# carkod/binquant

Hardware: AMD Instinct MI355X
Metric: symbol-candles/s for full indicator set (14 fp64 columns) (higher is better)
Workload: dtype f64; 1 GPU; configs[3]: 100000 symbols x 10000 candles, symbol-sharded over 1 GPU(s) (100000 symbols x 10000 candles on rank 0); symbols=100000, symbols_per_gpu=100000, candles=10000, parallelism=symbol-sharded x1, no data-path collective

## Files before the change

### binquant_amd/csrc/bq_device.h

```cpp
#pragma once
#include <hip/hip_runtime.h>
#include <math.h>
#include <stdint.h>

namespace bq {

constexpr int WAVE = 64;

__device__ __forceinline__ double qnan() { return __builtin_nan(""); }

__device__ __forceinline__ double win_val(double x) { return x - x == 0.0 ? x : qnan(); }
__device__ __forceinline__ bool win_ok(double x) { return x - x == 0.0; }

__device__ __forceinline__ uint64_t order_key(double v) {
  const uint64_t u = (uint64_t)__double_as_longlong(v);
  return (u >> 63) ? ~u : (u | 0x8000000000000000ull);
}

__device__ __forceinline__ double key_value(uint64_t k) {
  const uint64_t u = (k >> 63) ? (k & 0x7fffffffffffffffull) : ~k;
  return __longlong_as_double((long long)u);
}

struct dd {
// ... 115 lines not shown
__device__ __forceinline__ int wave_scan_max_dpp(int x, int lane) {
  x = max(x, dpp_i32<DPP_ROW_SHR1>(x));
  x = max(x, dpp_i32<DPP_ROW_SHR2>(x));
  x = max(x, dpp_i32<DPP_ROW_SHR4>(x));
  x = max(x, dpp_i32<DPP_ROW_SHR8>(x));
  const int r0 = __builtin_amdgcn_readlane(x, 15);
  const int r1 = max(r0, __builtin_amdgcn_readlane(x, 31));
  const int r2 = max(r1, __builtin_amdgcn_readlane(x, 47));
  const int row = lane >> 4;
  const int c = row == 0 ? 0 : (row == 1 ? r0 : (row == 2 ? r1 : r2));
  return max(x, c);
}

template <int NB>
__device__ __forceinline__ double pow_bits(const double* apow, int n) {
  double r = 1.0;
#pragma unroll
  for (int j = 0; j < NB; ++j)
    if (n & (1 << j)) r *= apow[j];
  return r;
}

__device__ __forceinline__ double wave_scan_affine_dpp(double b, const double* apow, int lane) {
  b = fma(apow[0], dpp_f64<DPP_ROW_SHR1>(b), b);
  b = fma(apow[1], dpp_f64<DPP_ROW_SHR2>(b), b);
  b = fma(apow[2], dpp_f64<DPP_ROW_SHR4>(b), b);
  b = fma(apow[3], dpp_f64<DPP_ROW_SHR8>(b), b);
  const double c1 = readlane_f64(b, 15);
  const double c2 = fma(apow[4], c1, readlane_f64(b, 31));
  const double c3 = fma(apow[4], c2, readlane_f64(b, 47));
  const int row = lane >> 4;
  if (row > 0) {
    const double c = row == 1 ? c1 : (row == 2 ? c2 : c3);
    b = fma(pow_bits<5>(apow, (lane & 15) + 1), c, b);
  }
  return b;
}

__device__ __forceinline__ double wave_scan_affine_dpp_rp(double b, const double* apow, double rp, int lane) {
  b = fma(apow[0], dpp_f64<DPP_ROW_SHR1>(b), b);
  b = fma(apow[1], dpp_f64<DPP_ROW_SHR2>(b), b);
  b = fma(apow[2], dpp_f64<DPP_ROW_SHR4>(b), b);
  b = fma(apow[3], dpp_f64<DPP_ROW_SHR8>(b), b);
  const double c1 = readlane_f64(b, 15);
  const double c2 = fma(apow[4], c1, readlane_f64(b, 31));
  const double c3 = fma(apow[4], c2, readlane_f64(b, 47));
  const int row = lane >> 4;
  if (row > 0) {
    const double c = row == 1 ? c1 : (row == 2 ? c2 : c3);
    b = fma(rp, c, b);
  }
  return b;
}

__device__ __forceinline__ double gain_of(double d) { return d > 0.0 ? d : 0.0; }
__device__ __forceinline__ double loss_of(double d) { return d < 0.0 ? -d : 0.0; }

__device__ __forceinline__ double true_range(double h, double l, double pc) {
  double a = h - l;
  double b = fabs(h - pc);
  double c = fabs(l - pc);
  return fmax(a, fmax(b, c));
}

__device__ __forceinline__ double ohlc4(double o, double h, double l, double c) {
  return (((o + h) + l) + c) / 4.0;
}

__device__ __forceinline__ double typical_price(double h, double l, double c) {
  return ((h + l) + c) / 3.0;
}

__device__ __forceinline__ double oscillator(double a, double b) {
  return (100.0 * a) / (a + b);
}

__device__ __forceinline__ double div_exact(double x, double n, double r) {
  double q = x * r;
  const double e = fma(-q, n, x);
  return fma(e, r, q);
}

__device__ __forceinline__ double div_count(double x, double n, double r) {
  if (__builtin_expect(fabs(x) < 0x1p-960 && x != 0.0, 0)) return x / n;
  const double q = x * r;
  const double c = fma(fma(-q, n, x), r, q);
  return ((x == 0.0) | !(fabs(q) <= __DBL_MAX__)) ? q : c;
}

__device__ __forceinline__ double rcp_nr(double v) {
  double r = __builtin_amdgcn_rcp(v);
  r = fma(r, fma(-v, r, 1.0), r);
  return fma(r, fma(-v, r, 1.0), r);
}

__device__ __forceinline__ double log_return(double c, double p) {
  const double m = c / p;
  const double d = m - 1.0;
  if (__builtin_expect(!(fabs(d) <= 0.125), 0)) return log(m);
  const double s = d * rcp_nr(2.0 + d), z = s * s;
  double r = 1.0 / 15.0;
  r = fma(r, z, 1.0 / 13.0);
  r = fma(r, z, 1.0 / 11.0);
  r = fma(r, z, 1.0 / 9.0);
  r = fma(r, z, 1.0 / 7.0);
  r = fma(r, z, 1.0 / 5.0);
  r = fma(r, z, 1.0 / 3.0);
  return (2.0 * s) * fma(r, z, 1.0);
}

__device__ __forceinline__ double sqrt_nr(double v) {
  const double r = __builtin_amdgcn_rsq(v);
  const double s = v * r;
  const double h = 0.5 * r;
  const double e = fma(-s, s, v);
  const double q = fma(h, e, s);
  return v > 0.0 ? q : 0.0;
}

constexpr int STG_PITCH = WAVE + 2;

typedef unsigned int bq_u32x2 __attribute__((__vector_size__(8)));

template <int CT>
__device__ __forceinline__ void stage_load(const double* __restrict__ base, int64_t ld, int64_t sym0, int64_t S,
                                           int t0, int T, int lane, double (&r)[CT]) {
#pragma unroll
  for (int k = 0; k < CT; ++k) {
    const int e = lane + WAVE * k;
    const int64_t s = sym0 + e / CT;
    const int t = t0 + e % CT;
    const int64_t sc = s < S ? s : S - 1;
    const int tc = t < 0 ? 0 : t < T ? t : T - 1;
    const double v = base[sc * ld + tc];
    r[k] = (s < S && t >= 0 && t < T) ? v : qnan();
  }
}

template <int CT>
__device__ __forceinline__ void stage_put(double* lds, int lane, const double (&r)[CT]) {
#pragma unroll
  for (int k = 0; k < CT; ++k) {
    const int e = lane + WAVE * k;
    lds[(e % CT) * STG_PITCH + e / CT] = r[k];
  }
}

template <int CT, typename OutT>
__device__ __forceinline__ void stage_store(const double* lds, OutT* __restrict__ base, int64_t ld, int64_t sym0,
                                            int64_t S, int t0, int T, int lane) {
  const int64_t rows = S - sym0 < WAVE ? S - sym0 : WAVE;
  const int nbytes = base ? (int)(rows * ld * (int64_t)sizeof(OutT)) : 0;
  const __amdgpu_buffer_rsrc_t rs =
      __builtin_amdgcn_make_buffer_rsrc(base ? base + sym0 * ld : nullptr, 0, nbytes, 0x00020000);
#pragma unroll
  for (int k = 0; k < CT; ++k) {
    const int e = lane + WAVE * k;
    const int r = e / CT;
    const int t = t0 + e % CT;
    const bool ok = r < rows && t < T;
    const unsigned off = ok ? (unsigned)(((int64_t)r * ld + t) * (int64_t)sizeof(OutT)) : (unsigned)nbytes;
    const double v = lds[(e % CT) * STG_PITCH + r];
    if constexpr (sizeof(OutT) == 1)
      __builtin_amdgcn_raw_buffer_store_b8((unsigned char)(OutT)v, rs, off, 0, 0);
    else
      __builtin_amdgcn_raw_buffer_store_b64(__builtin_bit_cast(bq_u32x2, (double)(OutT)v), rs, off, 0, 0);
  }
}

__device__ __forceinline__ int lower_bound_i64(const int64_t* __restrict__ ts, int n, int64_t key) {
  int lo = 0, hi = n;
  while (lo < hi) {
    const int mid = (lo + hi) >> 1;
    if (ts[mid] < key) lo = mid + 1;
    else hi = mid;
  }
  return lo;
}

__device__ __forceinline__ int lower_bound_guess(const int64_t* __restrict__ ts, int n, int64_t key, int64_t t0v,
                                                 int64_t step) {
  if (step > 0) {
    int64_t g = key <= t0v ? 0 : (key - t0v + step - 1) / step;
    g = g > n ? n : g;
    const bool ok = (g == 0 || ts[g - 1] < key) && (g == n || ts[g] >= key);
    if (ok) return (int)g;
  }
  return lower_bound_i64(ts, n, key);
}

__device__ __forceinline__ double safe_pct(double cur, double prev) {
  if (prev == 0.0) return 0.0;
  return (cur - prev) / fabs(prev);
}


typedef double dbl2 __attribute__((ext_vector_type(2)));

union DwordsOf2 {
  dbl2 d;
  unsigned u[4];
};

__device__ __forceinline__ void swap_halves(dbl2& a, dbl2& b) {
  DwordsOf2 x, y;
  x.d = a;
  y.d = b;
#pragma unroll
  for (int i = 0; i < 4; ++i) {
    const auto r = __builtin_amdgcn_permlane32_swap(x.u[i], y.u[i], false, false);
    x.u[i] = r[0];
    y.u[i] = r[1];
  }
  a = x.d;
  b = y.d;
}

__device__ __forceinline__ void swap_rows(dbl2& a, dbl2& b) {
  DwordsOf2 x, y;
  x.d = a;
  y.d = b;
#pragma unroll
  for (int i = 0; i < 4; ++i) {
    const auto r = __builtin_amdgcn_permlane16_swap(x.u[i], y.u[i], false, false);
    x.u[i] = r[0];
    y.u[i] = r[1];
  }
  a = x.d;
  b = y.d;
}

template <int K>
__device__ __forceinline__ void line_exchange(dbl2 (&p)[K / 2]) {
  static_assert(K == 4 || K == 8, "line_exchange: 4 or 8 candles per lane");
  if constexpr (K == 4) {
    swap_halves(p[0], p[1]);
  } else {
    swap_halves(p[0], p[2]);
    swap_halves(p[1], p[3]);
    swap_rows(p[0], p[1]);
    swap_rows(p[2], p[3]);
  }
}

template <int K>
__device__ __forceinline__ int line_offset(int lane) {
  if constexpr (K == 4) return lane < 32 ? 4 * lane : 4 * (lane - 32) + 2;
  else return 8 * (lane & 15) + 2 * (lane >> 4);
}


template <int K>
__device__ __forceinline__ void store_lines(double* __restrict__ row_, int tb, int T, bool vec, const double (&x)[K],
                                            bool full = false) {
  typedef __attribute__((address_space(1))) double gd;
  typedef __attribute__((address_space(1))) dbl2 gd2;
  gd* row = (gd*)row_;
  if (vec) {
    dbl2 p[K / 2];
#pragma unroll
    for (int j = 0; j < K / 2; ++j) p[j] = dbl2{x[2 * j], x[2 * j + 1]};
    line_exchange<K>(p);
    const int lane = __lane_id();
    const int t = tb - K * lane + line_offset<K>(lane);
#pragma unroll
    for (int m = 0; m < K / 2; ++m) {
      const int u = t + 128 * m;
      if (full || u + 2 <= T) __builtin_nontemporal_store(p[m], reinterpret_cast<gd2*>(row + u));
      else if (u < T) row[u] = p[m].x;
    }
  } else {
#pragma unroll
    for (int k = 0; k < K; ++k)
      if (tb + k < T) row[tb + k] = x[k];
  }
}


template <bool UNROLL, typename F>
__device__ __forceinline__ void walk_window(int lo, F&& f) {
  if constexpr (UNROLL) {
#pragma unroll
    for (int x = lo; x <= 0; ++x) f(x);
  } else {
    for (int x = lo; x <= 0; ++x) f(x);
  }
}


template <int K>
__device__ __forceinline__ void line_unexchange(dbl2 (&p)[K / 2]) {
  static_assert(K == 4 || K == 8, "line_unexchange: 4 or 8 candles per lane");
  if constexpr (K == 4) {
    swap_halves(p[0], p[1]);
  } else {
    swap_rows(p[0], p[1]);
    swap_rows(p[2], p[3]);
    swap_halves(p[0], p[2]);
    swap_halves(p[1], p[3]);
  }
}

template <int K>
__device__ __forceinline__ void load_pieces(const double* __restrict__ row, int tb, int T, double (&x)[K],
                                            double fill) {
  const int lane = __lane_id();
  const int t = tb - K * lane + line_offset<K>(lane);
#pragma unroll
  for (int m = 0; m < K / 2; ++m) {
    const int u = t + 128 * m;
    if (u + 2 <= T) {
      const dbl2 v = *reinterpret_cast<const dbl2*>(row + u);
      x[2 * m] = v.x;
      x[2 * m + 1] = v.y;
    } else {
      x[2 * m] = u < T ? row[u] : fill;
      x[2 * m + 1] = fill;
    }
  }
}

template <int K>
__device__ __forceinline__ void line_unexchange_x(double (&x)[K]) {
  dbl2 p[K / 2];
#pragma unroll
  for (int m = 0; m < K / 2; ++m) p[m] = dbl2{x[2 * m], x[2 * m + 1]};
  line_unexchange<K>(p);
#pragma unroll
  for (int m = 0; m < K / 2; ++m) {
    x[2 * m] = p[m].x;
    x[2 * m + 1] = p[m].y;
  }
}

}
```

### binquant_amd/csrc/bq_enrich.hip

```cpp
#include "bq_rowtile.h"
#include "binquant_amd.h"

#include <stddef.h>
#include <string.h>

#include <type_traits>

namespace bq {

#ifndef BQ_EN_NT
#define BQ_EN_NT 256
#endif
#ifndef BQ_EN_K
#define BQ_EN_K 4
#endif
#ifndef BQ_EN_NTSTORE
#define BQ_EN_NTSTORE 1
#endif
#ifndef BQ_EN_SWIZZLE
#define BQ_EN_SWIZZLE 0
#endif
#ifndef BQ_EN_WPS
#define BQ_EN_WPS 3
#endif
constexpr int EN_NT = BQ_EN_NT;
constexpr int EN_NW = EN_NT / WAVE;
constexpr int EN_K = BQ_EN_K;
constexpr int EN_TT = EN_NT * EN_K;
constexpr int EN_LK = EN_K == 2 ? 1 : EN_K == 4 ? 2 : 3;
constexpr int EN_H = 128;
constexpr int EN_R = EN_H + EN_TT;
static_assert(EN_K % 2 == 0 && EN_TT >= EN_H && EN_K * WAVE > BQ_MAX_WINDOW, "tile shape");

#ifndef BQ_EN_LDSPERM
#define BQ_EN_LDSPERM 1
#endif
#if BQ_EN_LDSPERM
#define LX(i) ((((i) & (EN_K - 1)) * (EN_R / EN_K)) + ((i) >> EN_LK))
#define RS(x) (lb + LX(x))
#define RS1(x) (pb / EN_K + LX(x))
#else
#define LX(i) (i)
#define RS(x) (pb + (x))
#define RS1(x) (pb + (x))
#endif
static_assert(!BQ_EN_LDSPERM || ((1 << EN_LK) == EN_K && EN_R % EN_K == 0), "LX: power-of-two candles per lane");

enum { E_FAST = 0, E_SLOW, E_SIG, E_0, E_1, NE };

struct Pow {
  double a0, a1, p, q, a2, a3, a4;
};

__host__ __device__ __forceinline__ Pow pow_mul(const Pow& T, const Pow& U) {
  Pow r;
  r.a0 = T.a0 * U.a0;
  r.a1 = T.a1 * U.a1;
  r.p = fma(T.p, U.a0, T.a2 * U.p);
  r.q = fma(T.q, U.a1, T.a2 * U.q);
  r.a2 = T.a2 * U.a2;
  r.a3 = T.a3 * U.a3;
  r.a4 = T.a4 * U.a4;
  return r;
}

struct EmaHost {
  double al[NE], om[NE], den[NE], la[NE], lb[NE];
  Pow step;
  Pow wstep[6];
  Pow wave[EN_NW + 1];
};

struct EnrichArgs {
  EmaHost ema;
  const double* in[BQ_NUM_INPUTS];
  double* out[BQ_NUM_ENRICH_COLS];
  int64_t ld_in, ld_out;
  int64_t S, swz;
  int T;
  int ma[3];
  int rsi_w, bb_w, bb_ddof, atr_w, twap_w, mfi_w;
  int span[NE];
  double bb_k;
  double inv_ma[3], inv_rsi, inv_bb, inv_bb_dv, inv_atr, inv_twap;
};

struct EmaConsts {
  double al[NE], om[NE], den[NE], la[NE], lb[NE];
  Pow step;
  Pow wstep[6];
  Pow wave[EN_NW + 1];
  Pow lane[WAVE];
};
static_assert(sizeof(EmaHost) % sizeof(double) == 0 && offsetof(EmaConsts, lane) == sizeof(EmaHost),
              "EmaConsts begins with EmaHost's layout");

static EmaHost ema_consts(const int (&span)[NE]) {
  EmaHost E;
  for (int e = 0; e < NE; ++e) {
    const double com = ((double)span[e] - 1.0) / 2.0;
    const double al = 1.0 / (1.0 + com);
    E.al[e] = al;
    E.om[e] = 1.0 - al;
    E.den[e] = E.om[e] + al;
    E.la[e] = E.om[e] / E.den[e];
    E.lb[e] = al / E.den[e];
  }
  Pow m;
  m.a0 = E.la[E_FAST];
  m.a1 = E.la[E_SLOW];
  m.a2 = E.la[E_SIG];
  m.p = E.lb[E_SIG] * E.la[E_FAST];
  m.q = -(E.lb[E_SIG] * E.la[E_SLOW]);
  m.a3 = E.la[E_0];
  m.a4 = E.la[E_1];
  E.step = m;
  Pow mk = m;
  for (int k = 1; k < EN_K; ++k) mk = pow_mul(m, mk);
  for (int j = 0; j < 6; ++j) {
    E.wstep[j] = mk;
    mk = pow_mul(mk, mk);
  }
  Pow r = {1.0, 1.0, 0.0, 0.0, 1.0, 1.0, 1.0};
  const Pow w64 = pow_mul(E.wstep[5], E.wstep[5]);
  for (int k = 0; k <= EN_NW; ++k) {
    E.wave[k] = r;
    r = pow_mul(w64, r);
  }
  return E;
}

__device__ __forceinline__ void pow_apply(const Pow& A, const double (&v)[NE], double (&r)[NE]) {
  r[E_FAST] = A.a0 * v[E_FAST];
  r[E_SLOW] = A.a1 * v[E_SLOW];
  r[E_SIG] = fma(A.p, v[E_FAST], fma(A.q, v[E_SLOW], A.a2 * v[E_SIG]));
  r[E_0] = A.a3 * v[E_0];
  r[E_1] = A.a4 * v[E_1];
}

template <bool DIV, bool SEL = false>
__device__ __forceinline__ double ema_step(double y, double x, const EmaConsts& E, int e) {
  static_assert(!(DIV && SEL), "SEL: without the divide only");
  if constexpr (SEL) {
    const double n = E.om[e] * y + E.al[e] * x;
    return y != x ? n : y;
  } else {
    if (y != x) {
      y = E.om[e] * y + E.al[e] * x;
      if (DIV) y = y / E.den[e];
    }
    return y;
  }
}

__device__ __forceinline__ double sel_f64(bool c, double a, double b) {
  const int hi = c ? __double2hiint(a) : __double2hiint(b);
  const int lo = c ? __double2loint(a) : __double2loint(b);
  return __hiloint2double(hi, lo);
}

typedef __attribute__((address_space(1))) double gdouble;
typedef __attribute__((address_space(1))) dbl2 gdbl2;

#ifndef BQ_EN_SWAPST
#define BQ_EN_SWAPST 1
#endif

__device__ __forceinline__ void put2(gdouble* row, int t, int T, bool full, dbl2 v) {
  if (full || t + 2 <= T) {
#if BQ_EN_NTSTORE
    __builtin_nontemporal_store(v, reinterpret_cast<gdbl2*>(row + t));
#else
    *reinterpret_cast<gdbl2*>(row + t) = v;
#endif
  } else if (t < T) {
    row[t] = v.x;
  }
}

__device__ __forceinline__ void store4(double* __restrict__ row_, int tb, int T, bool vec, const double (&x)[EN_K],
                                       bool full = false) {
  gdouble* row = (gdouble*)row_;
#if BQ_EN_SWAPST
  if constexpr (EN_K == 4) {
    if (vec) {
      union {
        dbl2 d;
        unsigned u[4];
      } a, b;
      a.d = dbl2{x[0], x[1]};
      b.d = dbl2{x[2], x[3]};
#pragma unroll
      for (int i = 0; i < 4; ++i) {
        const auto r = __builtin_amdgcn_permlane32_swap(a.u[i], b.u[i], false, false);
        a.u[i] = r[0];
        b.u[i] = r[1];
      }
      const int lane = __lane_id();
      const int ta = lane < 32 ? tb : tb - 126;
      put2(row, ta, T, full, a.d);
      put2(row, ta + 128, T, full, b.d);
      return;
    }
  }
#endif
  if (vec && tb + EN_K <= T) {
    gdbl2* p = reinterpret_cast<gdbl2*>(row + tb);
#pragma unroll
    for (int j = 0; j < EN_K / 2; ++j) {
#if BQ_EN_NTSTORE
      __builtin_nontemporal_store(dbl2{x[2 * j], x[2 * j + 1]}, p + j);
#else
      p[j] = dbl2{x[2 * j], x[2 * j + 1]};
#endif
    }
  } else {
#pragma unroll
    for (int k = 0; k < EN_K; ++k)
      if (tb + k < T) row[tb + k] = x[k];
  }
}

struct Tile {
  double o[EN_K], h[EN_K], l[EN_K], c[EN_K], v[EN_K];
  double ph, pl, pc;
};

#ifndef BQ_EN_LINELOAD
#define BQ_EN_LINELOAD 0
#endif

__device__ __forceinline__ void load_tile(const EnrichArgs& A, int64_t row, int tb, bool vin, Tile& t) {
  const int T = A.T;
  if (BQ_EN_LINELOAD && vin) {
    load_pieces<EN_K>(A.in[BQ_OPEN] + row, tb, T, t.o, 0.0);
    load_pieces<EN_K>(A.in[BQ_HIGH] + row, tb, T, t.h, 0.0);
    load_pieces<EN_K>(A.in[BQ_LOW] + row, tb, T, t.l, 0.0);
    load_pieces<EN_K>(A.in[BQ_CLOSE] + row, tb, T, t.c, 0.0);
    load_pieces<EN_K>(A.in[BQ_VOLUME] + row, tb, T, t.v, 0.0);
  } else {
    load_lane<EN_K, false>(A.in[BQ_OPEN] + row, tb, T, vin, t.o);
    load_lane<EN_K, false>(A.in[BQ_HIGH] + row, tb, T, vin, t.h);
    load_lane<EN_K, false>(A.in[BQ_LOW] + row, tb, T, vin, t.l);
    load_lane<EN_K, false>(A.in[BQ_CLOSE] + row, tb, T, vin, t.c);
    load_lane<EN_K, false>(A.in[BQ_VOLUME] + row, tb, T, vin, t.v);
  }
  if (tb >= 1 && tb <= T) {
    t.ph = A.in[BQ_HIGH][row + tb - 1];
    t.pl = A.in[BQ_LOW][row + tb - 1];
    t.pc = A.in[BQ_CLOSE][row + tb - 1];
  } else {
    t.ph = t.pl = t.pc = qnan();
  }
}

__device__ __forceinline__ void tile_arrived(bool vin, Tile& t) {
  if (BQ_EN_LINELOAD && vin) {
    line_unexchange_x<EN_K>(t.o);
    line_unexchange_x<EN_K>(t.h);
    line_unexchange_x<EN_K>(t.l);
    line_unexchange_x<EN_K>(t.c);
    line_unexchange_x<EN_K>(t.v);
  }
}

typedef dbl2 __attribute__((aligned(8))) dbl2u;

__device__ __forceinline__ void load_tile_clamped(const EnrichArgs& A, int64_t row, int tb, Tile& t) {
  const int T = A.T;
  int64_t u[EN_K / 2];
#pragma unroll
  for (int j = 0; j < EN_K / 2; ++j) u[j] = row + min(tb + 2 * j, T - 2);
  auto field = [&](const double* __restrict__ f, double (&x)[EN_K]) {
#pragma unroll
    for (int j = 0; j < EN_K / 2; ++j) {
      const dbl2u a = *reinterpret_cast<const dbl2u*>(f + u[j]);
      x[2 * j] = a.x;
      x[2 * j + 1] = a.y;
    }
  };
  field(A.in[BQ_OPEN], t.o);
  field(A.in[BQ_HIGH], t.h);
  field(A.in[BQ_LOW], t.l);
  field(A.in[BQ_CLOSE], t.c);
  field(A.in[BQ_VOLUME], t.v);
  const int64_t n = row + min(tb - 1, T - 1);
  t.ph = A.in[BQ_HIGH][n];
  t.pl = A.in[BQ_LOW][n];
  t.pc = A.in[BQ_CLOSE][n];
}

__device__ __forceinline__ void tile_tail_select(int tb, int T, Tile& t) {
  auto field = [&](double (&x)[EN_K]) {
#pragma unroll
    for (int j = 0; j < EN_K / 2; ++j) {
      const int u = tb + 2 * j;
      const bool both = u + 2 <= T, one = u < T;
      x[2 * j] = both ? x[2 * j] : (one ? x[2 * j + 1] : 0.0);
      x[2 * j + 1] = both ? x[2 * j + 1] : 0.0;
    }
  };
  field(t.o);
  field(t.h);
  field(t.l);
  field(t.c);
  field(t.v);
  if (tb > T) t.ph = t.pl = t.pc = qnan();
}

template <bool GEN_, bool WARM_, bool RANGE_, bool PREF_, bool SEL_>
struct TileMode {
  static constexpr bool GEN = GEN_, WARM = WARM_, RANGE = RANGE_, PREF = PREF_, SEL = SEL_;
};

template <bool DEF>
__device__ __forceinline__ int win_of(int def, int v) {
  return DEF ? def : __builtin_amdgcn_readfirstlane(v);
}

struct WinAgg {
  double sum, first;
  bool ok, same;
};

template <typename F>
__device__ __forceinline__ WinAgg win_agg(F val, int t, int w) {
  WinAgg a = {0.0, 0.0, t >= w - 1, true};
  if (!a.ok) return a;
  a.first = val(t - w + 1);
  for (int j = t - w + 1; j <= t; ++j) {
    const double x = val(j);
    if (!__builtin_isfinite(x)) {
      a.ok = false;
      return a;
    }
    a.same &= x == a.first;
    a.sum += x;
  }
  return a;
}

__device__ __forceinline__ double ewm_gap_step(double& wt, double& old, double x, double al, double om) {
  const bool obs = __builtin_isfinite(x);
  if (wt == wt) {
    old *= om;
    if (obs) {
      if (wt != x) {
        wt = old * wt + al * x;
        wt /= (old + al);
      }
      old = 1.0;
    }
  } else if (obs) {
    wt = x;
  }
  return wt;
}

__device__ __forceinline__ void enrich_row_missing(const EnrichArgs& P, const EmaConsts& E, int64_t irow, int64_t orow,
                                                double* bc, double* b0, double* b1, double* b2, double* b3) {
  const int tid = threadIdx.x, T = P.T;
  const double* __restrict__ po = P.in[BQ_OPEN] + irow;
  const double* __restrict__ ph = P.in[BQ_HIGH] + irow;
  const double* __restrict__ pl = P.in[BQ_LOW] + irow;
  const double* __restrict__ pc = P.in[BQ_CLOSE] + irow;
  const double* __restrict__ pv = P.in[BQ_VOLUME] + irow;
  auto C = [&](int j) { return j >= 0 ? pc[j] : qnan(); };
  auto TP = [&](int j) { return j >= 0 ? typical_price(ph[j], pl[j], pc[j]) : qnan(); };
  auto put = [&](int col, int t, double v) {
    if (P.out[col]) P.out[col][orow + t] = v;
  };
  auto mean_of = [&](const WinAgg& a, int w) { return !a.ok ? qnan() : (a.same ? a.first : a.sum / (double)w); };
  for (int t = tid; t < T; t += EN_NT) {
    for (int i = 0; i < 3; ++i)
      if (P.out[BQ_MA_FAST + i]) put(BQ_MA_FAST + i, t, mean_of(win_agg(C, t, P.ma[i]), P.ma[i]));
    if (P.out[BQ_BB_UPPER] || P.out[BQ_BB_MID] || P.out[BQ_BB_LOWER]) {
      const int w = P.bb_w;
      const WinAgg a = win_agg(C, t, w);
      double m = qnan(), sd = qnan();
      if (a.ok) {
        m = mean_of(a, w);
        double ss = 0.0;
        if (!a.same)
          for (int j = t - w + 1; j <= t; ++j) {
            const double d = pc[j] - m;
            ss += d * d;
          }
        sd = w - P.bb_ddof > 0 ? sqrt(ss / (double)(w - P.bb_ddof)) : qnan();
      }
      put(BQ_BB_MID, t, m);
      put(BQ_BB_UPPER, t, m + (P.bb_k * sd));
      put(BQ_BB_LOWER, t, m - (P.bb_k * sd));
    }
    if (P.out[BQ_TWAP])
      put(BQ_TWAP, t, mean_of(win_agg([&](int j) { return ohlc4(po[j], ph[j], pl[j], pc[j]); }, t, P.twap_w),
                              P.twap_w));
    if (P.out[BQ_ATR])
      put(BQ_ATR, t, mean_of(win_agg([&](int j) { return true_range(ph[j], pl[j], C(j - 1)); }, t, P.atr_w),
                             P.atr_w));
    if (P.out[BQ_RSI]) {
      const int w = P.rsi_w;
      const WinAgg g = win_agg([&](int j) { const double d = C(j) - C(j - 1); return d > 0.0 ? d : 0.0; }, t, w);
      const WinAgg l = win_agg([&](int j) { const double d = C(j) - C(j - 1); return d < 0.0 ? -d : 0.0; }, t, w);
      const double rs = mean_of(g, w) / mean_of(l, w);
      put(BQ_RSI, t, 100.0 - (100.0 / (1.0 + rs)));
    }
    if (P.out[BQ_MFI]) {
      const int w = P.mfi_w;
      const WinAgg p = win_agg([&](int j) { const double tp = TP(j); return tp > TP(j - 1) ? tp * pv[j] : 0.0; }, t, w);
      const WinAgg n = win_agg([&](int j) { const double tp = TP(j); return tp < TP(j - 1) ? tp * pv[j] : 0.0; }, t, w);
      const double ps = p.ok ? p.sum : qnan(), ns = n.ok ? n.sum : qnan();
      put(BQ_MFI, t, 100.0 - (100.0 / (1.0 + ps / ns)));
    }
  }
  const bool ema = P.out[BQ_MACD] || P.out[BQ_MACD_SIGNAL] || P.out[BQ_EMA_FAST] || P.out[BQ_EMA_SLOW];
  if (!ema) return;
  double wf = qnan(), of = 1.0, ws = qnan(), os = 1.0, wg = qnan(), og = 1.0, we = qnan(), oe = 1.0;
  for (int c0 = 0; c0 < T; c0 += EN_TT) {
    const int n = min(EN_TT, T - c0);
    __syncthreads();
    for (int i = tid; i < n; i += EN_NT) bc[i] = pc[c0 + i];
    __syncthreads();
    if (tid == 0) {
      for (int i = 0; i < n; ++i) {
        const double x = bc[i];
        const double f = ewm_gap_step(wf, of, x, E.al[E_FAST], E.om[E_FAST]);
        const double s = ewm_gap_step(ws, os, x, E.al[E_SLOW], E.om[E_SLOW]);
        const double m = f - s;
        b0[i] = m;
        b1[i] = ewm_gap_step(wg, og, m, E.al[E_SIG], E.om[E_SIG]);
      }
    } else if (tid == WAVE || tid == 2 * WAVE) {
      const int e = tid == WAVE ? E_0 : E_1;
      double* dst = tid == WAVE ? b2 : b3;
      for (int i = 0; i < n; ++i) dst[i] = ewm_gap_step(we, oe, bc[i], E.al[e], E.om[e]);
    }
    __syncthreads();
    for (int i = tid; i < n; i += EN_NT) {
      put(BQ_MACD, c0 + i, b0[i]);
      put(BQ_MACD_SIGNAL, c0 + i, b1[i]);
      put(BQ_EMA_FAST, c0 + i, b2[i]);
      put(BQ_EMA_SLOW, c0 + i, b3[i]);
    }
  }
}

template <bool DIV, bool VOUT, bool DEF, bool HOT = false>
__global__ __launch_bounds__(EN_NT, BQ_EN_WPS) void enrich_kernel(const EnrichArgs A, int vec_in) {
  static_assert(!HOT || (!DIV && VOUT && DEF && !BQ_EN_LINELOAD && EN_K == 4), "HOT: the common call only");
  __shared__ double sP[EN_R];
  __shared__ double sC[EN_R];
  __shared__ double sTR[EN_R];
  __shared__ double sO4[EN_R];
  __shared__ double sMF[EN_R];
  __shared__ double sWh[EN_NW], sWl[EN_NW];
  __shared__ double sWe[EN_NW][NE];
  __shared__ int sWlc[EN_NW];
  __shared__ double sEcar[NE];
  __shared__ int sLcar, sMiss;
  __shared__ EmaConsts E;
  __shared__ EnrichArgs sA;

  const int tid = threadIdx.x, lane = tid & (WAVE - 1);
  const int w = __builtin_amdgcn_readfirstlane(tid / WAVE);
  const int64_t sym = BQ_EN_SWIZZLE ? ((int64_t)blockIdx.x * A.swz) % A.S : (int64_t)blockIdx.x;
  const int64_t irow = sym * A.ld_in;
  const int64_t orow = sym * A.ld_out;
  const int T = A.T;
  const bool vin = HOT || vec_in != 0, vout = VOUT;

  Tile nx;
  load_tile(A, irow, EN_K * tid, vin, nx);

  {
    const double* src = reinterpret_cast<const double*>(&A.ema);
    double* dst = reinterpret_cast<double*>(&E);
    for (int i = tid; i < (int)(sizeof(EmaHost) / sizeof(double)); i += EN_NT) dst[i] = src[i];
  }
  if (tid < WAVE) {
    Pow r = {1.0, 1.0, 0.0, 0.0, 1.0, 1.0, 1.0};
    for (int j = 0; j < 6; ++j)
      if (tid & (1 << j)) r = pow_mul(A.ema.wstep[j], r);
    E.lane[tid] = r;
  }
  if (tid < NE) sEcar[tid] = 0.0;
  if (tid == 0) {
    sLcar = -1;
    sMiss = 0;
    sA = A;
  }
  if (tid < EN_H) {
    sP[LX(tid)] = 0.0;
    sC[LX(tid)] = qnan();
    sTR[LX(tid)] = 0.0;
    sO4[LX(tid)] = 0.0;
    sMF[LX(tid)] = 0.0;
  }
  __syncthreads();

  if (tid == 0) {
    const double x0 = nx.c[0];
    sEcar[E_FAST] = sEcar[E_SLOW] = sEcar[E_0] = sEcar[E_1] = x0;
    sEcar[E_SIG] = 0.0;
  }

  const int pb = EN_H + EN_K * tid;
  int lcl[EN_K];
  double Ploc[EN_K];
  double y[NE];
  auto ploc = [&](int k) -> double {
    if constexpr (HOT) return sP[RS1(k)];
    else return Ploc[k];
  };

  constexpr bool DBUF = HOT;
  int par = 0;
  auto ecar_in = [&]() -> const double* { return DBUF && par ? sWe[EN_NW - 1] : sEcar; };
  auto ecar_out = [&]() -> double* { return par ? sEcar : sWe[EN_NW - 1]; };

  auto tile = [&](auto mode, const int t0) {
    using M = decltype(mode);
    const int tb = t0 + EN_K * tid;
    const EnrichArgs& P = sA;
    auto has = [&](int col) { return HOT || P.out[col] != nullptr; };
    Tile cu = nx;
    if constexpr (M::SEL) tile_tail_select(tb, T, cu);
    else tile_arrived(vin, cu);
    if constexpr (M::GEN) {
      if (t0 + EN_TT < T) load_tile(A, irow, tb + EN_TT, vin, nx);
    }

    {
      bool miss = false;
      double pc = cu.pc;
      double tpp = typical_price(cu.ph, cu.pl, cu.pc);
      int run = -1;
#pragma unroll
      for (int k = 0; k < EN_K; ++k) {
        const int t = tb + k;
        const double c = cu.c[k];
        const double tp = typical_price(cu.h[k], cu.l[k], c);
        const double mf = tp * cu.v[k];
        const double o4 = ohlc4(cu.o[k], cu.h[k], cu.l[k], c);
        miss |= !__builtin_isfinite(o4) | !__builtin_isfinite(mf);
        sC[RS1(k)] = c;
        sTR[RS1(k)] = true_range(cu.h[k], cu.l[k], pc);
        sO4[RS1(k)] = o4;
        sMF[RS1(k)] = tp > tpp ? mf : (tp < tpp ? -mf : 0.0);
        if (t == 0 || c != pc) run = t;
        lcl[k] = run;
        pc = c;
        tpp = tp;
      }
      if (__builtin_amdgcn_ballot_w64(miss)) sMiss = 1;
    }
    if constexpr (M::PREF) load_tile_clamped(A, irow, tb + EN_TT, nx);
    {
      dd tot = {0.0, 0.0};
#pragma unroll
      for (int k = 0; k < EN_K; ++k) tot = dd_add1(tot, cu.c[k]);
      const dd inc = wave_scan_dd_dpp(tot, lane);
      if (lane == WAVE - 1) {
        sWh[w] = inc.hi;
        sWl[w] = inc.lo;
      }
      dd acc = {dpp_f64<DPP_WAVE_SHR1>(inc.hi), dpp_f64<DPP_WAVE_SHR1>(inc.lo)};
#pragma unroll
      for (int k = 0; k < EN_K; ++k) {
        acc = dd_add1(acc, cu.c[k]);
        Ploc[k] = dd_round(acc);
        sP[RS1(k)] = Ploc[k];
      }
    }
    double ex[NE];
    {
      double b[NE] = {0.0, 0.0, 0.0, 0.0, 0.0};
#pragma unroll
      for (int k = 0; k < EN_K; ++k) {
        const double x = cu.c[k];
        b[E_FAST] = fma(E.la[E_FAST], b[E_FAST], E.lb[E_FAST] * x);
        b[E_SLOW] = fma(E.la[E_SLOW], b[E_SLOW], E.lb[E_SLOW] * x);
        b[E_SIG] = fma(E.la[E_SIG], b[E_SIG], E.lb[E_SIG] * (b[E_FAST] - b[E_SLOW]));
        b[E_0] = fma(E.la[E_0], b[E_0], E.lb[E_0] * x);
        b[E_1] = fma(E.la[E_1], b[E_1], E.lb[E_1] * x);
      }
#define BQ_EMA_STEP(CTRL, J)                                     \
  {                                                              \
    double v[NE], r[NE];                                         \
    _Pragma("unroll") for (int e = 0; e < NE; ++e) v[e] = dpp_f64<CTRL>(b[e]); \
    pow_apply(E.wstep[J], v, r);                                 \
    _Pragma("unroll") for (int e = 0; e < NE; ++e) b[e] += r[e]; \
  }
      BQ_EMA_STEP(DPP_ROW_SHR1, 0)
      BQ_EMA_STEP(DPP_ROW_SHR2, 1)
      BQ_EMA_STEP(DPP_ROW_SHR4, 2)
      BQ_EMA_STEP(DPP_ROW_SHR8, 3)
#undef BQ_EMA_STEP
      {
        double c1[NE], c2[NE], c3[NE], r[NE];
#pragma unroll
        for (int e = 0; e < NE; ++e) c1[e] = readlane_f64(b[e], 15);
        pow_apply(E.wstep[4], c1, r);
#pragma unroll
        for (int e = 0; e < NE; ++e) c2[e] = r[e] + readlane_f64(b[e], 31);
        pow_apply(E.wstep[4], c2, r);
#pragma unroll
        for (int e = 0; e < NE; ++e) c3[e] = r[e] + readlane_f64(b[e], 47);
        const int row = lane >> 4;
        double c[NE];
#pragma unroll
        for (int e = 0; e < NE; ++e) {
          const double a1 = c1[e], a2 = c2[e], a3 = c3[e];
          c[e] = row == 1 ? a1 : (row == 2 ? a2 : a3);
        }
        pow_apply(E.lane[(lane & 15) + 1], c, r);
#pragma unroll
        for (int e = 0; e < NE; ++e) b[e] = sel_f64(row > 0, b[e] + r[e], b[e]);
      }
      if (lane == WAVE - 1 && (!DBUF || w < EN_NW - 1)) {
#pragma unroll
        for (int e = 0; e < NE; ++e) sWe[w][e] = b[e];
      }
#pragma unroll
      for (int e = 0; e < NE; ++e) ex[e] = dpp_f64<DPP_WAVE_SHR1>(b[e]);
    }
    int lpre;
    {
      const int inc = wave_scan_max_dpp(lcl[EN_K - 1] + 1, lane);
      if (lane == WAVE - 1) sWlc[w] = inc - 1;
      lpre = dpp_i32<DPP_WAVE_SHR1>(inc) - 1;
    }
    __syncthreads();

    double wbw = 0.0, wbp = 0.0;
    {
      dd acc = {0.0, 0.0};
#pragma unroll
      for (int u = 0; u < EN_NW; ++u) {
        const double base = dd_round(acc);
        wbw = u == w ? base : wbw;
        wbp = u + 1 == w ? base : wbp;
        if (u + 1 < EN_NW) acc = dd_add(acc, dd{sWh[u], sWl[u]});
      }
    }
    {
      int carry = max(sLcar, lpre);
      int wl[EN_NW - 1];
#pragma unroll
      for (int u = 0; u < EN_NW - 1; ++u) wl[u] = sWlc[u];
#pragma unroll
      for (int u = 0; u < EN_NW - 1; ++u) carry = u < w ? max(carry, wl[u]) : carry;
#pragma unroll
      for (int k = 0; k < EN_K; ++k) lcl[k] = max(lcl[k], carry);
    }
    {
      double C[NE];
#pragma unroll
      for (int e = 0; e < NE; ++e) C[e] = ecar_in()[e];
      const Pow W1 = E.wave[1];
#pragma unroll
      for (int u = 0; u < EN_NW - 1; ++u) {
        if (u < w) {
          double r[NE];
          pow_apply(W1, C, r);
#pragma unroll
          for (int e = 0; e < NE; ++e) C[e] = r[e] + sWe[u][e];
        }
      }
      double r[NE];
      pow_apply(E.lane[lane], C, r);
#pragma unroll
      for (int e = 0; e < NE; ++e) y[e] = ex[e] + r[e];
    }

    {
      double mfast[EN_K], msig[EN_K], e0[EN_K], e1[EN_K];
#pragma unroll
      for (int k = 0; k < EN_K; ++k) {
        const double x = cu.c[k];
        y[E_FAST] = ema_step<DIV, HOT>(y[E_FAST], x, E, E_FAST);
        y[E_SLOW] = ema_step<DIV, HOT>(y[E_SLOW], x, E, E_SLOW);
        y[E_SIG] = ema_step<DIV, HOT>(y[E_SIG], y[E_FAST] - y[E_SLOW], E, E_SIG);
        y[E_0] = ema_step<DIV, HOT>(y[E_0], x, E, E_0);
        y[E_1] = ema_step<DIV, HOT>(y[E_1], x, E, E_1);
        mfast[k] = y[E_FAST] - y[E_SLOW];
        msig[k] = y[E_SIG];
        e0[k] = y[E_0];
        e1[k] = y[E_1];
      }
      if constexpr (DBUF) {
        if (tid == EN_NT - 1) {
#pragma unroll
          for (int e = 0; e < NE; ++e) ecar_out()[e] = y[e];
        }
      }
      const bool whole = M::GEN ? t0 + EN_TT <= T : !M::RANGE;
      if (has(BQ_MACD)) store4(P.out[BQ_MACD] + orow, tb, T, vout, mfast, whole);
      if (has(BQ_MACD_SIGNAL)) store4(P.out[BQ_MACD_SIGNAL] + orow, tb, T, vout, msig, whole);
      if (has(BQ_EMA_FAST)) store4(P.out[BQ_EMA_FAST] + orow, tb, T, vout, e0, whole);
      if (has(BQ_EMA_SLOW)) store4(P.out[BQ_EMA_SLOW] + orow, tb, T, vout, e1, whole);
    }

    const int wstart = EN_H + EN_K * WAVE * w;
    auto windows = [&](auto nowarmc, auto fullstc) {
      constexpr bool NOWARM = decltype(nowarmc)::value;
      constexpr bool FULLST = decltype(fullstc)::value;
      const int gstart = EN_H - t0;
      int lb = pb / EN_K;
      if constexpr (HOT) asm volatile("" : "+v"(lb));
      (void)lb;
      auto warm = [&](int t, int win) { return !NOWARM && t < win - 1; };
      auto put = [&](double* col, const double (&x)[EN_K]) {
        if (FULLST) store4(col + orow, tb, T, true, x, true);
        else store4(col + orow, tb, T, vout, x);
      };
      auto cmean = [&](int win, double inv, int k) -> double {
        const int t = tb + k, p = pb + k;
        const int q = p - win;
        const double base = q >= wstart ? wbw : wbp;
        const double m = div_exact((ploc(k) + wbw) - (sP[RS(k - win)] + base), (double)win, inv);
        const double v = lcl[k] <= t - win + 1 ? cu.c[k] : m;
        return warm(t, win) ? qnan() : v;
      };
      double res[EN_K];
#pragma unroll
      for (int i = 0; i < 3; ++i) {
        if (has(BQ_MA_FAST + i)) {
          const int win = win_of<DEF>(i == 0 ? 7 : (i == 1 ? 25 : 100), P.ma[i]);
          const double inv = P.inv_ma[i];
#pragma unroll
          for (int k = 0; k < EN_K; ++k) res[k] = cmean(win, inv, k);
          put(P.out[BQ_MA_FAST + i], res);
        }
      }
      if (has(BQ_BB_UPPER) || has(BQ_BB_MID) || has(BQ_BB_LOWER)) {
        double up[EN_K], mid[EN_K], lo[EN_K];
        const int win = win_of<DEF>(20, P.bb_w);
        const double bk = P.bb_k, invw = P.inv_bb, invdv = P.inv_bb_dv;
        const bool okdv = win > P.bb_ddof;
        const double r = cu.c[0];
        double s1 = 0.0, s2 = 0.0;
        walk_window<DEF && NOWARM>(NOWARM ? 1 - win : max(1 - win, gstart - pb), [&](int x) {
          const double d = sC[RS(x)] - r;
          s1 += d;
          s2 = fma(d, d, s2);
        });
#pragma unroll
        for (int k = 0; k < EN_K; ++k) {
          const int t = tb + k, p = pb + k;
          if (k > 0) {
            const double dn = cu.c[k] - r;
            const double cold = sC[RS(k - win)];
            const double dol = (NOWARM || p - win >= gstart) ? cold - r : 0.0;
            s1 = (s1 + dn) - dol;
            s2 = fma(-dol, dol, fma(dn, dn, s2));
          }
          const double m = cmean(win, invw, k);
          const double var = (s2 - s1 * s1 * invw) * invdv;
          const double sdv = lcl[k] <= t - win + 1 ? 0.0 : sqrt_nr(var);
          const double sd = (warm(t, win) || !okdv) ? qnan() : sdv;
          mid[k] = m;
          up[k] = m + bk * sd;
          lo[k] = m - bk * sd;
        }
        if (has(BQ_BB_UPPER)) put(P.out[BQ_BB_UPPER], up);
        if (has(BQ_BB_MID)) put(P.out[BQ_BB_MID], mid);
        if (has(BQ_BB_LOWER)) put(P.out[BQ_BB_LOWER], lo);
      }
      if (has(BQ_RSI)) {
        const int win = win_of<DEF>(14, P.rsi_w);
        double A = 0.0, prev = sC[RS(-win)];
        int nup = 0, ndn = 0;
        walk_window<DEF>(1 - win, [&](int x) {
          const double c = sC[RS(x)], d = c - prev;
          A += fmax(fabs(d), 0.0);
          nup += d > 0.0;
          ndn += d < 0.0;
          prev = c;
        });
#pragma unroll
        for (int k = 0; k < EN_K; ++k) {
          const int t = tb + k, p = pb + k;
          if (k > 0) {
            const double d = cu.c[k] - cu.c[k - 1];
            const double dold = sC[RS(k - win)] - sC[RS(k - win - 1)];
            A = (A + fabs(d)) - fmax(fabs(dold), 0.0);
            nup += (d > 0.0) - (dold > 0.0);
            ndn += (d < 0.0) - (dold < 0.0);
          }
          const double D = cu.c[k] - sC[NOWARM ? RS(k - win) : (p - win >= gstart ? RS(k - win) : LX(gstart))];
          double v = 50.0 * (1.0 + D / A);
          v = nup == 0 ? 0.0 : v;
          v = ndn == 0 ? 100.0 : v;
          v = (nup == 0 && ndn == 0) ? qnan() : v;
          res[k] = warm(t, win) ? qnan() : v;
        }
        put(P.out[BQ_RSI], res);
      }
      auto smean = [&](const double* Q, int defw, int win_, double inv, bool nonneg) {
        const int win = win_of<DEF>(defw, win_);
        const double wd = (double)win;
        double sum = 0.0, pq = qnan();
        int run = 0;
        walk_window<DEF>(1 - win, [&](int x) {
          const double q = Q[RS(x)];
          sum += q;
          run = q == pq ? run + 1 : 1;
          pq = q;
        });
#pragma unroll
        for (int k = 0; k < EN_K; ++k) {
          const int t = tb + k;
          if (k > 0) {
            const double q = Q[RS(k)];
            sum = (sum + q) - Q[RS(k - win)];
            run = q == pq ? run + 1 : 1;
            pq = q;
          }
          const double m = div_exact(nonneg && sum < 0.0 ? 0.0 : sum, wd, inv);
          const double v = run >= win ? pq : m;
          res[k] = warm(t, win) ? qnan() : v;
        }
      };
      if (has(BQ_ATR)) {
        smean(sTR, 14, P.atr_w, P.inv_atr, true);
        put(P.out[BQ_ATR], res);
      }
      if (has(BQ_TWAP)) {
        smean(sO4, 12, P.twap_w, P.inv_twap, false);
        put(P.out[BQ_TWAP], res);
      }
      if (has(BQ_MFI)) {
        const int win = win_of<DEF>(14, P.mfi_w);
        double B = 0.0, F = 0.0;
        int nup = 0, ndn = 0;
        walk_window<DEF>(1 - win, [&](int x) {
          const double f = sMF[RS(x)];
          B += fabs(f);
          F += f;
          nup += f > 0.0;
          ndn += f < 0.0;
        });
#pragma unroll
        for (int k = 0; k < EN_K; ++k) {
          const int t = tb + k;
          if (k > 0) {
            const double f = sMF[RS(k)], fo = sMF[RS(k - win)];
            B = (B + fabs(f)) - fabs(fo);
            F = (F + f) - fo;
            nup += (f > 0.0) - (fo > 0.0);
            ndn += (f < 0.0) - (fo < 0.0);
          }
          double v = 50.0 * (1.0 + F / B);
          v = nup == 0 ? 0.0 : v;
          v = ndn == 0 ? 100.0 : v;
          res[k] = (warm(t, win) || (nup == 0 && ndn == 0)) ? qnan() : v;
        }
        put(P.out[BQ_MFI], res);
      }
    };
    if constexpr (M::GEN) {
      const bool full = t0 >= EN_H && t0 + EN_TT <= T && vout;
      if (full) windows(std::true_type{}, std::true_type{});
      else windows(std::false_type{}, std::false_type{});
    } else {
      windows(std::bool_constant<!M::WARM>{}, std::bool_constant<!M::RANGE>{});
    }
  };

  auto halo = [&]() {
    __syncthreads();
    const double plast = HOT ? sP[LX(EN_R - 1)] : __shfl(Ploc[EN_K - 1], WAVE - 1, WAVE);
    if (pb >= EN_TT) {
      double hp[EN_K], hc[EN_K], htr[EN_K], ho4[EN_K], hmf[EN_K];
#pragma unroll
      for (int k = 0; k < EN_K; ++k) {
        hp[k] = ploc(k) - plast;
        hc[k] = sC[RS1(k)];
        htr[k] = sTR[RS1(k)];
        ho4[k] = sO4[RS1(k)];
        hmf[k] = sMF[RS1(k)];
      }
#pragma unroll
      for (int k = 0; k < EN_K; ++k) {
        sP[RS1(k - EN_TT)] = hp[k];
        sC[RS1(k - EN_TT)] = hc[k];
        sTR[RS1(k - EN_TT)] = htr[k];
        sO4[RS1(k - EN_TT)] = ho4[k];
        sMF[RS1(k - EN_TT)] = hmf[k];
      }
    }
    if (tid == EN_NT - 1) {
      if constexpr (!DBUF) {
#pragma unroll
        for (int e = 0; e < NE; ++e) sEcar[e] = y[e];
      }
      sLcar = lcl[EN_K - 1];
    }
    if constexpr (DBUF) par ^= 1;
  };

  if constexpr (!HOT) {
    for (int t0 = 0; t0 < T; t0 += EN_TT) {
      tile(TileMode<true, false, false, false, false>{}, t0);
      if (t0 + EN_TT >= T) break;
      halo();
    }
  } else if (T < EN_TT) {
    tile(TileMode<false, true, true, false, false>{}, 0);
  } else {
    tile(TileMode<false, true, false, true, false>{}, 0);
    int t0 = EN_TT;
    for (; t0 + EN_TT <= T; t0 += EN_TT) {
      halo();
      tile(TileMode<false, false, false, true, false>{}, t0);
    }
    if (t0 < T) {
      halo();
      tile(TileMode<false, false, true, false, true>{}, t0);
    }
  }
  __syncthreads();
  if (sMiss) enrich_row_missing(sA, E, irow, orow, sC, sP, sTR, sO4, sMF);
}

static bool window_ok(int w) { return w >= 1 && w <= BQ_MAX_WINDOW; }

}

extern "C" {

void bq_default_params(bq_params* p) {
  if (!p) return;
  memset(p, 0, sizeof(*p));
  p->ma_periods[0] = 7;
  p->ma_periods[1] = 25;
  p->ma_periods[2] = 100;
  p->macd_fast = 12;
  p->macd_slow = 26;
  p->macd_signal = 9;
  p->rsi_window = 14;
  p->bb_window = 20;
  p->bb_ddof = 1;
  p->atr_window = 14;
  p->twap_window = 12;
  p->ema_spans[0] = 20;
  p->ema_spans[1] = 50;
  p->mfi_window = 14;
  p->bb_k = 2.0;
}

const char* bq_version(void) { return "binquant_amd 0.2.0 (gfx950)"; }

int bq_device_arch(char* buf, int buflen) {
  if (!buf || buflen <= 0) return BQ_EINVAL;
  int dev = 0;
  if (hipGetDevice(&dev) != hipSuccess) return BQ_EHIP;
  hipDeviceProp_t prop;
  if (hipGetDeviceProperties(&prop, dev) != hipSuccess) return BQ_EHIP;
  strncpy(buf, prop.gcnArchName, (size_t)buflen - 1);
  buf[buflen - 1] = 0;
  return BQ_OK;
}

int bq_enrich(const double* const* in, int64_t S, int64_t T, int64_t ld_in, const bq_params* params,
              double* const* out, int64_t ld_out, void* stream) {
  using namespace bq;
  if (!in || !out || S < 0 || T < 0 || ld_in < T || ld_out < T || T > (int64_t)0x7fffffff - 2 * EN_TT ||
      S > 0x7fffffff)
    return BQ_EINVAL;
  bq_params dp;
  if (!params) {
    bq_default_params(&dp);
    params = &dp;
  }
  const bq_params& P = *params;
  for (int i = 0; i < 3; ++i)
    if (!window_ok(P.ma_periods[i])) return BQ_EINVAL;
  if (!window_ok(P.rsi_window) || !window_ok(P.bb_window) || !window_ok(P.atr_window) ||
      !window_ok(P.twap_window) || !window_ok(P.mfi_window) || P.bb_ddof < 0 || P.macd_fast < 1 ||
      P.macd_slow < 1 || P.macd_signal < 1 || P.ema_spans[0] < 1 || P.ema_spans[1] < 1)
    return BQ_EINVAL;
  EnrichArgs A;
  memset(&A, 0, sizeof(A));
  bool any_out = false;
  for (int i = 0; i < BQ_NUM_INPUTS; ++i) {
    if (!in[i]) return BQ_EINVAL;
    A.in[i] = in[i];
  }
  for (int i = 0; i < BQ_NUM_ENRICH_COLS; ++i) {
    A.out[i] = out[i];
    any_out |= out[i] != nullptr;
  }
  if (S == 0 || T == 0 || !any_out) return BQ_OK;
  A.ld_in = ld_in;
  A.ld_out = ld_out;
  A.T = (int)T;
  A.S = S;
  A.swz = 1;
  {
    auto gcd = [](int64_t a, int64_t b) {
      while (b) {
        const int64_t t = a % b;
        a = b;
        b = t;
      }
      return a;
    };
    const int64_t primes[] = {7919, 7927, 7933, 7937, 7949, 104729};
    for (int64_t p : primes)
      if (S > 1 && gcd(p % S, S) == 1) {
        A.swz = p % S;
        break;
      }
  }
  for (int i = 0; i < 3; ++i) A.ma[i] = P.ma_periods[i];
  A.rsi_w = P.rsi_window;
  A.bb_w = P.bb_window;
  A.bb_ddof = P.bb_ddof;
  A.atr_w = P.atr_window;
  A.twap_w = P.twap_window;
  A.mfi_w = P.mfi_window;
  A.bb_k = P.bb_k;
  for (int i = 0; i < 3; ++i) A.inv_ma[i] = 1.0 / (double)P.ma_periods[i];
  A.inv_rsi = 1.0 / (double)P.rsi_window;
  A.inv_bb = 1.0 / (double)P.bb_window;
  A.inv_bb_dv = P.bb_window > P.bb_ddof ? 1.0 / (double)(P.bb_window - P.bb_ddof) : 0.0;
  A.inv_atr = 1.0 / (double)P.atr_window;
  A.inv_twap = 1.0 / (double)P.twap_window;
  A.span[E_FAST] = P.macd_fast;
  A.span[E_SLOW] = P.macd_slow;
  A.span[E_SIG] = P.macd_signal;
  A.span[E_0] = P.ema_spans[0];
  A.span[E_1] = P.ema_spans[1];
  A.ema = ema_consts(A.span);

  const int vin = vec_rows(in, BQ_NUM_INPUTS, ld_in), vout = vec_rows(out, BQ_NUM_ENRICH_COLS, ld_out);

  bool div = false;
  for (int e = 0; e < NE; ++e) {
    const double com = ((double)A.span[e] - 1.0) / 2.0;
    const double al = 1.0 / (1.0 + com);
    div |= ((1.0 - al) + al) != 1.0;
  }
  const dim3 grid((unsigned)S), block(EN_NT);
  hipStream_t st = (hipStream_t)stream;
  const bool def = P.ma_periods[0] == 7 && P.ma_periods[1] == 25 && P.ma_periods[2] == 100 && P.rsi_window == 14 &&
                   P.bb_window == 20 && P.atr_window == 14 && P.twap_window == 12 && P.mfi_window == 14;
  bool hot = def && !div && vout && vin && !BQ_EN_LINELOAD && EN_K == 4;
  for (int i = 0; i < BQ_NUM_ENRICH_COLS; ++i) hot &= out[i] != nullptr;
#define BQ_EN_LAUNCH(D, V, F) hipLaunchKernelGGL((enrich_kernel<D, V, F>), grid, block, 0, st, A, vin)
  if (hot) {
    if constexpr (!BQ_EN_LINELOAD && EN_K == 4)
      hipLaunchKernelGGL((enrich_kernel<false, true, true, true>), grid, block, 0, st, A, vin);
  } else if (def) {
    if (div && vout) BQ_EN_LAUNCH(true, true, true);
    else if (div) BQ_EN_LAUNCH(true, false, true);
    else if (vout) BQ_EN_LAUNCH(false, true, true);
    else BQ_EN_LAUNCH(false, false, true);
  } else {
    if (div && vout) BQ_EN_LAUNCH(true, true, false);
    else if (div) BQ_EN_LAUNCH(true, false, false);
    else if (vout) BQ_EN_LAUNCH(false, true, false);
    else BQ_EN_LAUNCH(false, false, false);
  }
#undef BQ_EN_LAUNCH
  return hipGetLastError() == hipSuccess ? BQ_OK : BQ_EHIP;
}

}
```

Before: 40.63 billion symbol-candles/s.

## Use line-coalesced prefetch loads and DPP neighbor exchange in hot enrich path

The hot kernel's clamped prefetch now loads each field in 128-element-strided line pieces (mirroring the permlane32 store layout) and unexchanges them in registers after arrival, so wave loads cover contiguous cache lines. The previous-candle high/low/close values are fetched once per wave and passed between lanes with DPP shift-right instead of each lane loading its own neighbor. Typical price also switches to an exact-division helper by default. This costs extra register shuffles and lane permutes per tile, and the line-unexchange now runs in all arrival modes of the hot path.

```diff
diff --git a/binquant_amd/csrc/bq_device.h b/binquant_amd/csrc/bq_device.h
--- a/binquant_amd/csrc/bq_device.h
+++ b/binquant_amd/csrc/bq_device.h
@@ -441,25 +441,6 @@
 }
 
 template <int K>
-__device__ __forceinline__ void load_pieces(const double* __restrict__ row, int tb, int T, double (&x)[K],
-                                            double fill) {
-  const int lane = __lane_id();
-  const int t = tb - K * lane + line_offset<K>(lane);
-#pragma unroll
-  for (int m = 0; m < K / 2; ++m) {
-    const int u = t + 128 * m;
-    if (u + 2 <= T) {
-      const dbl2 v = *reinterpret_cast<const dbl2*>(row + u);
-      x[2 * m] = v.x;
-      x[2 * m + 1] = v.y;
-    } else {
-      x[2 * m] = u < T ? row[u] : fill;
-      x[2 * m + 1] = fill;
-    }
-  }
-}
-
-template <int K>
 __device__ __forceinline__ void line_unexchange_x(double (&x)[K]) {
   dbl2 p[K / 2];
 #pragma unroll
diff --git a/binquant_amd/csrc/bq_enrich.hip b/binquant_amd/csrc/bq_enrich.hip
--- a/binquant_amd/csrc/bq_enrich.hip
+++ b/binquant_amd/csrc/bq_enrich.hip
@@ -178,6 +178,8 @@
   }
 }
 
+__device__ __forceinline__ int tile_line_base(int tb) { return __lane_id() < 32 ? tb : tb - 126; }
+
 __device__ __forceinline__ void store4(double* __restrict__ row_, int tb, int T, bool vec, const double (&x)[EN_K],
                                        bool full = false) {
   gdouble* row = (gdouble*)row_;
@@ -196,8 +198,7 @@
         a.u[i] = r[0];
         b.u[i] = r[1];
       }
-      const int lane = __lane_id();
-      const int ta = lane < 32 ? tb : tb - 126;
+      const int ta = tile_line_base(tb);
       put2(row, ta, T, full, a.d);
       put2(row, ta + 128, T, full, b.d);
       return;
@@ -226,25 +227,13 @@
   double ph, pl, pc;
 };
 
-#ifndef BQ_EN_LINELOAD
-#define BQ_EN_LINELOAD 0
-#endif
-
 __device__ __forceinline__ void load_tile(const EnrichArgs& A, int64_t row, int tb, bool vin, Tile& t) {
   const int T = A.T;
-  if (BQ_EN_LINELOAD && vin) {
-    load_pieces<EN_K>(A.in[BQ_OPEN] + row, tb, T, t.o, 0.0);
-    load_pieces<EN_K>(A.in[BQ_HIGH] + row, tb, T, t.h, 0.0);
-    load_pieces<EN_K>(A.in[BQ_LOW] + row, tb, T, t.l, 0.0);
-    load_pieces<EN_K>(A.in[BQ_CLOSE] + row, tb, T, t.c, 0.0);
-    load_pieces<EN_K>(A.in[BQ_VOLUME] + row, tb, T, t.v, 0.0);
-  } else {
-    load_lane<EN_K, false>(A.in[BQ_OPEN] + row, tb, T, vin, t.o);
-    load_lane<EN_K, false>(A.in[BQ_HIGH] + row, tb, T, vin, t.h);
-    load_lane<EN_K, false>(A.in[BQ_LOW] + row, tb, T, vin, t.l);
-    load_lane<EN_K, false>(A.in[BQ_CLOSE] + row, tb, T, vin, t.c);
-    load_lane<EN_K, false>(A.in[BQ_VOLUME] + row, tb, T, vin, t.v);
-  }
+  load_lane<EN_K, false>(A.in[BQ_OPEN] + row, tb, T, vin, t.o);
+  load_lane<EN_K, false>(A.in[BQ_HIGH] + row, tb, T, vin, t.h);
+  load_lane<EN_K, false>(A.in[BQ_LOW] + row, tb, T, vin, t.l);
+  load_lane<EN_K, false>(A.in[BQ_CLOSE] + row, tb, T, vin, t.c);
+  load_lane<EN_K, false>(A.in[BQ_VOLUME] + row, tb, T, vin, t.v);
   if (tb >= 1 && tb <= T) {
     t.ph = A.in[BQ_HIGH][row + tb - 1];
     t.pl = A.in[BQ_LOW][row + tb - 1];
@@ -254,23 +243,23 @@
   }
 }
 
-__device__ __forceinline__ void tile_arrived(bool vin, Tile& t) {
-  if (BQ_EN_LINELOAD && vin) {
-    line_unexchange_x<EN_K>(t.o);
-    line_unexchange_x<EN_K>(t.h);
-    line_unexchange_x<EN_K>(t.l);
-    line_unexchange_x<EN_K>(t.c);
-    line_unexchange_x<EN_K>(t.v);
-  }
-}
-
+#ifndef BQ_EN_HOTLINE
+#define BQ_EN_HOTLINE 1
+#endif
+#ifndef BQ_EN_WAVENB
+#define BQ_EN_WAVENB 1
+#endif
+#ifndef BQ_EN_TPDIV
+#define BQ_EN_TPDIV 0
+#endif
 typedef dbl2 __attribute__((aligned(8))) dbl2u;
-
-__device__ __forceinline__ void load_tile_clamped(const EnrichArgs& A, int64_t row, int tb, Tile& t) {
+constexpr int EN_PS = BQ_EN_HOTLINE ? 128 : 2;
+
+__device__ __forceinline__ void load_tile_clamped(const EnrichArgs& A, int64_t row, int tb, int tp, Tile& t) {
   const int T = A.T;
   int64_t u[EN_K / 2];
 #pragma unroll
-  for (int j = 0; j < EN_K / 2; ++j) u[j] = row + min(tb + 2 * j, T - 2);
+  for (int j = 0; j < EN_K / 2; ++j) u[j] = row + min(tp + EN_PS * j, T - 2);
   auto field = [&](const double* __restrict__ f, double (&x)[EN_K]) {
 #pragma unroll
     for (int j = 0; j < EN_K / 2; ++j) {
@@ -284,17 +273,18 @@
   field(A.in[BQ_LOW], t.l);
   field(A.in[BQ_CLOSE], t.c);
   field(A.in[BQ_VOLUME], t.v);
-  const int64_t n = row + min(tb - 1, T - 1);
+  const int nb = BQ_EN_WAVENB ? tb - EN_K * (int)__lane_id() : tb;
+  const int64_t n = row + min(nb - 1, T - 1);
   t.ph = A.in[BQ_HIGH][n];
   t.pl = A.in[BQ_LOW][n];
   t.pc = A.in[BQ_CLOSE][n];
 }
 
-__device__ __forceinline__ void tile_tail_select(int tb, int T, Tile& t) {
+__device__ __forceinline__ void tile_tail_select(int tp, int T, Tile& t) {
   auto field = [&](double (&x)[EN_K]) {
 #pragma unroll
     for (int j = 0; j < EN_K / 2; ++j) {
-      const int u = tb + 2 * j;
+      const int u = tp + EN_PS * j;
       const bool both = u + 2 <= T, one = u < T;
       x[2 * j] = both ? x[2 * j] : (one ? x[2 * j + 1] : 0.0);
       x[2 * j + 1] = both ? x[2 * j + 1] : 0.0;
@@ -305,7 +295,32 @@
   field(t.l);
   field(t.c);
   field(t.v);
-  if (tb > T) t.ph = t.pl = t.pc = qnan();
+}
+
+__device__ __forceinline__ double prev_lane_or(double keep, double x) {
+  const int lo = __builtin_amdgcn_update_dpp(__double2loint(keep), __double2loint(x), DPP_WAVE_SHR1, 0xF, 0xF, false);
+  const int hi = __builtin_amdgcn_update_dpp(__double2hiint(keep), __double2hiint(x), DPP_WAVE_SHR1, 0xF, 0xF, false);
+  return __hiloint2double(hi, lo);
+}
+
+template <bool TAIL>
+__device__ __forceinline__ void hot_tile_arrived(int tb, int tp, int T, Tile& t) {
+  if constexpr (TAIL) tile_tail_select(tp, T, t);
+#if BQ_EN_HOTLINE
+  line_unexchange_x<EN_K>(t.o);
+  line_unexchange_x<EN_K>(t.h);
+  line_unexchange_x<EN_K>(t.l);
+  line_unexchange_x<EN_K>(t.c);
+  line_unexchange_x<EN_K>(t.v);
+#endif
+#if BQ_EN_WAVENB
+  t.ph = prev_lane_or(t.ph, t.h[EN_K - 1]);
+  t.pl = prev_lane_or(t.pl, t.l[EN_K - 1]);
+  t.pc = prev_lane_or(t.pc, t.c[EN_K - 1]);
+#endif
+  if constexpr (TAIL) {
+    if (tb > T) t.ph = t.pl = t.pc = qnan();
+  }
 }
 
 template <bool GEN_, bool WARM_, bool RANGE_, bool PREF_, bool SEL_>
@@ -447,7 +462,7 @@
 
 template <bool DIV, bool VOUT, bool DEF, bool HOT = false>
 __global__ __launch_bounds__(EN_NT, BQ_EN_WPS) void enrich_kernel(const EnrichArgs A, int vec_in) {
-  static_assert(!HOT || (!DIV && VOUT && DEF && !BQ_EN_LINELOAD && EN_K == 4), "HOT: the common call only");
+  static_assert(!HOT || (!DIV && VOUT && DEF && EN_K == 4), "HOT: the common call only");
   __shared__ double sP[EN_R];
   __shared__ double sC[EN_R];
   __shared__ double sTR[EN_R];
@@ -524,22 +539,28 @@
     const EnrichArgs& P = sA;
     auto has = [&](int col) { return HOT || P.out[col] != nullptr; };
     Tile cu = nx;
-    if constexpr (M::SEL) tile_tail_select(tb, T, cu);
-    else tile_arrived(vin, cu);
+    constexpr bool ARRIVE = !M::GEN && !M::WARM;
+    const int tp = BQ_EN_HOTLINE ? tile_line_base(tb) : tb;
+    if constexpr (ARRIVE) hot_tile_arrived<M::SEL>(tb, tp, T, cu);
     if constexpr (M::GEN) {
       if (t0 + EN_TT < T) load_tile(A, irow, tb + EN_TT, vin, nx);
     }
 
     {
       bool miss = false;
+#if BQ_EN_TPDIV
+      auto tprice = [](double h, double l, double c) { return typical_price(h, l, c); };
+#else
+      auto tprice = [](double h, double l, double c) { return div_exact((h + l) + c, 3.0, 1.0 / 3.0); };
+#endif
       double pc = cu.pc;
-      double tpp = typical_price(cu.ph, cu.pl, cu.pc);
+      double tpp = tprice(cu.ph, cu.pl, cu.pc);
       int run = -1;
 #pragma unroll
       for (int k = 0; k < EN_K; ++k) {
         const int t = tb + k;
         const double c = cu.c[k];
-        const double tp = typical_price(cu.h[k], cu.l[k], c);
+        const double tp = tprice(cu.h[k], cu.l[k], c);
         const double mf = tp * cu.v[k];
         const double o4 = ohlc4(cu.o[k], cu.h[k], cu.l[k], c);
         miss |= !__builtin_isfinite(o4) | !__builtin_isfinite(mf);
@@ -554,7 +575,7 @@
       }
       if (__builtin_amdgcn_ballot_w64(miss)) sMiss = 1;
     }
-    if constexpr (M::PREF) load_tile_clamped(A, irow, tb + EN_TT, nx);
+    if constexpr (M::PREF) load_tile_clamped(A, irow, tb + EN_TT, tp + EN_TT, nx);
     {
       dd tot = {0.0, 0.0};
 #pragma unroll
@@ -1047,11 +1068,11 @@
   hipStream_t st = (hipStream_t)stream;
   const bool def = P.ma_periods[0] == 7 && P.ma_periods[1] == 25 && P.ma_periods[2] == 100 && P.rsi_window == 14 &&
                    P.bb_window == 20 && P.atr_window == 14 && P.twap_window == 12 && P.mfi_window == 14;
-  bool hot = def && !div && vout && vin && !BQ_EN_LINELOAD && EN_K == 4;
+  bool hot = def && !div && vout && vin && EN_K == 4;
   for (int i = 0; i < BQ_NUM_ENRICH_COLS; ++i) hot &= out[i] != nullptr;
 #define BQ_EN_LAUNCH(D, V, F) hipLaunchKernelGGL((enrich_kernel<D, V, F>), grid, block, 0, st, A, vin)
   if (hot) {
-    if constexpr (!BQ_EN_LINELOAD && EN_K == 4)
+    if constexpr (EN_K == 4)
       hipLaunchKernelGGL((enrich_kernel<false, true, true, true>), grid, block, 0, st, A, vin);
   } else if (def) {
     if (div && vout) BQ_EN_LAUNCH(true, true, true);
```

Result: faster. 41.47 billion symbol-candles/s (median of 6 runs) (+2.1%).
